# AllenNeuralDynamics/aind-smartspim-destripe

Hardware: AMD Instinct MI355X
Metric: 2048x2048 uint16 slices/s destriped (higher is better)
Workload: dtype f32

## Files before the change

### aind_smartspim_destripe_amd/csrc/dsx.hip

```cpp
#include <hip/hip_runtime.h>
#include <dlfcn.h>
#include <math.h>
#include <rccl/rccl.h>
#include <stdio.h>
#include <stdlib.h>
#include <string.h>

#include <string>
#include <vector>

#include "../../include/dsx.h"
#include "dsx_kernels.h"
#include "dsx_retile.h"
#include "dsx_rot90.h"
#include "dsx_pyramid.h"
#include "dsx_stackrank.h"
#include "dsx_volhist.h"
#include "dsx_project.h"
#include "dsx_wavelet.h"
#include "dsx_plan.h"
#include "dsx_chain.h"
#include "dsx_io.h"
#include "dsx_streaks.h"
#include "dsx_lightsheet.h"
// ... 230 lines not shown
  static bool done[64] = {};
  int dev = 0;
  (void)hipGetDevice(&dev);
  if (done[dev & 63]) return hipSuccess;
  const hipError_t e = hipFuncSetAttribute((const void*)KERN, hipFuncAttributeMaxDynamicSharedMemorySize, (int)bytes);
  if (e == hipSuccess) done[dev & 63] = true;
  return e;
}

template <int CPL, int GF = -1, int NT = -1, int HALO = -1, int PLAN = 0>
hipError_t launch_rowfilter(const DsxTuning& t, const dsx::RowArgs& a, int npairs, int nb, hipStream_t s) {
  if (hipError_t e = raise_lds_limit<dsx::k_rowfilter<CPL, GF, NT, HALO, PLAN>>()) return e;
  const dsx::RowLaunch g = dsx::rowfilter_launch(t, CPL, a.M, npairs);
  hipLaunchKernelGGL((dsx::k_rowfilter<CPL, GF, NT, HALO, PLAN>), dim3(g.grid_x, nb), dim3(64 * g.wpb), g.lds, s, a);
  return hipGetLastError();
}

hipError_t launch_rowfilter_wide(const dsx::RowArgs& a, int npairs, int nb, hipStream_t s) {
  if (hipError_t e = raise_lds_limit<dsx::k_rowfilter_wide>(dsx::kWideMaxLen * sizeof(float2))) return e;
  if (a.M > dsx::kWideMaxLen || a.w >= 65536) return hipErrorInvalidValue;
  hipLaunchKernelGGL(dsx::k_rowfilter_wide, dim3(npairs, nb), dim3(dsx::kWideThreads), (size_t)a.M * sizeof(float2), s, a);
  return hipGetLastError();
}

template <int ID>
hipError_t launch_rowfilter_plan(const DsxTuning& t, const dsx::RowArgs& a, int npairs, int nb, hipStream_t s) {
  constexpr dsx::RowPlan p = dsx::row_plan(ID);
  return launch_rowfilter<p.cpl, p.gf, p.nt, p.halo, ID>(t, a, npairs, nb, s);
}

hipError_t dispatch_rowfilter(const DsxTuning& t, const dsx::RowArgs& a, int npairs, int nb, hipStream_t s) {
  const dsx::RowClass c = dsx::classify_row(a.M, a.w, a.K, a.npass, a.radix);
  if (c.wide) return launch_rowfilter_wide(a, npairs, nb, s);
  switch (c.cpl) {
    case 2: return launch_rowfilter<2>(t, a, npairs, nb, s);
    case 4: return launch_rowfilter<4>(t, a, npairs, nb, s);
    case 6: return launch_rowfilter<6>(t, a, npairs, nb, s);
    case 10: return launch_rowfilter<10>(t, a, npairs, nb, s);
    case 18:
      if (c.plan == 1) return launch_rowfilter_plan<1>(t, a, npairs, nb, s);
      if (c.gf == 4) return launch_rowfilter<18, 4, 1, 0>(t, a, npairs, nb, s);
      if (c.plan == 2) return launch_rowfilter_plan<2>(t, a, npairs, nb, s);
      if (c.gf == 2) return launch_rowfilter<18, 2, 1, 1>(t, a, npairs, nb, s);
      if (c.plan == 5) return launch_rowfilter_plan<5>(t, a, npairs, nb, s);
      if (c.plan == 6) return launch_rowfilter_plan<6>(t, a, npairs, nb, s);
      return launch_rowfilter<18>(t, a, npairs, nb, s);
    default:
      if (c.plan == 3) return launch_rowfilter_plan<3>(t, a, npairs, nb, s);
      if (c.plan == 4) return launch_rowfilter_plan<4>(t, a, npairs, nb, s);
      return launch_rowfilter<36>(t, a, npairs, nb, s);
  }
}

template <int ID>
hipError_t launch_rowfinal_plan(const dsx::RowFinalArgs& a, int nb, hipStream_t s) {
  constexpr dsx::RowPlan p = dsx::row_plan(ID);
  constexpr auto kernel = dsx::k_rowfinal<p.cpl, p.gf, p.nt, p.halo, ID>;
  if (hipError_t e = raise_lds_limit<kernel>()) return e;
  const dsx::RowLaunch g = dsx::rowfinal_launch(a.r.M, a.f.hout);
  hipLaunchKernelGGL(kernel, dim3(g.grid_x, nb), dim3(64 * g.wpb), g.lds, s, a);
  return hipGetLastError();
}

hipError_t launch_rowfinal(int plan, const dsx::RowFinalArgs& a, int nb, hipStream_t s) {
  if (plan == 1) return launch_rowfinal_plan<1>(a, nb, s);
  if (plan == 3) return launch_rowfinal_plan<3>(a, nb, s);
  if (plan == 4) return launch_rowfinal_plan<4>(a, nb, s);
  return hipErrorInvalidValue;
}

hipError_t launch_rowfilter_multi(const dsx::RowMultiArgs& a_in, const int* npairs, int nb, hipStream_t s) {
  if (hipError_t e = raise_lds_limit<dsx::k_rowfilter_multi<6>>()) return e;
  dsx::RowMultiArgs a = a_in;
  int M[dsx::kRowMultiMax];
  for (int i = 0; i < a.nlev; ++i) M[i] = a.lv[i].M;
  const dsx::RowLaunch g = dsx::row_multi_launch(a.nlev, npairs, M, a.blk_end);
  hipLaunchKernelGGL(dsx::k_rowfilter_multi<6>, dim3(g.grid_x, nb), dim3(64 * g.wpb), g.lds, s, a);
  return hipGetLastError();
}

hipError_t launch_rowfilter_pack(const DsxTuning& t, const dsx::RowMultiArgs& m, const int* npairs, int nb, hipStream_t s) {
  if (hipError_t e = raise_lds_limit<dsx::k_rowfilter_pack<6>>()) return e;
  dsx::RowPackArgs a;
  memset(&a, 0, sizeof(a));
  a.nlev = m.nlev;
  int M[dsx::kRowMultiMax];
  for (int i = 0; i < m.nlev; ++i) {
    a.lv[i] = m.lv[i];
    M[i] = m.lv[i].M;
    a.pack[i] = dsx::row_pack_factor(t, m.lv[i].M, m.lv[i].npass, m.lv[i].radix);
  }
  const dsx::RowLaunch g = dsx::row_pack_launch(t, a.nlev, npairs, M, a.pack, a.blk_end);
  hipLaunchKernelGGL(dsx::k_rowfilter_pack<6>, dim3(g.grid_x, nb), dim3(64 * g.wpb), g.lds, s, a);
  return hipGetLastError();
}

struct Chain {
  dsx_ctx* ctx;
  const CohortView& v;
  dsx::ChainShape sh;
  const void* d_in;
  int in_dtype, nb;
  void* d_out;
  int out_dtype;
};

struct Skips {
  int hist, row, from;
};
Skips skips(const DsxTuning& t) {
#ifdef DSX_DIAG
// ... 273 lines not shown
    a.out_plane_stride = (long long)p.Hout * p.Wout;
    a.hout = p.Hout; a.wout = p.Wout;
    a.out_dtype = (c.out_dtype == DSX_U16) ? 0 : 1;
    a.flat = ctx->d_flat;
    a.dark = ctx->d_dark;
    a.dark_ld = ctx->dark_w;
  }
}

int stage_inverse(const Chain& c, const dsx::RowArgs& row1) {
  dsx_ctx* ctx = c.ctx;
  const dsx::Plan& p = ctx->plan;
  const CohortView& v = c.v;
  const dsx::ChainShape& sh = c.sh;
  hipStream_t s = v.stream;
  const int L = p.L, nb = c.nb;
  for (int l = L - 1; l >= (L > 0 ? 0 : -1); --l) {
    if (sh.fuse21 && l == 1) continue;
    if (l >= skips(ctx->tune).from) continue;
    const bool last = (l <= 0);
    LaunchScope ls(ctx, last ? KC_FINAL : KC_INV);
    if (sh.generic) {
      dsx::GenInvArgs g;
      fill_inv(g, c, l);
      g.F = ctx->wl_len;
      memcpy(g.lo, ctx->wl[2], sizeof(float) * ctx->wl_len);
      memcpy(g.hi, ctx->wl[3], sizeof(float) * ctx->wl_len);
      const dim3 gg((g.wout + dsx::kGenOW - 1) / dsx::kGenOW, (g.hout + dsx::kGenOH - 1) / dsx::kGenOH, nb);
      auto kern = level_kernel(last, c.in_dtype, dsx::k_inv_gen<2>, dsx::k_inv_gen<0>, dsx::k_inv_gen<1>);
      hipLaunchKernelGGL(kern, gg, dim3(256), dsx::gen_inv_lds_bytes(g.F), s, g);
      DSX_HIP(hipGetLastError());
      continue;
    }
    dsx::FinalArgs f;
    fill_inv(f, c, l);
    if (!last) f.ws_out = v.ws;
    f.ablate = ctx->ablate;
    const dsx::MarchLaunch m = dsx::inv_launch(sh, ctx->tune, ctx->cus, nb, l, f.hout, f.wout);
    f.nstrips = m.nstrips; f.nseg = m.nseg; f.rows_per_seg = m.rows_per_seg;
    const bool fused = sh.fuse21 && last;
    if (last && sh.split_inv) DSX_HIP(hipStreamWaitEvent(s, v.ev[3], 0));
    if (fused) {
      const dsx::LevelPlan& l2 = p.lv[1];
      f.c2_off = l2.aa_off; f.d2_off = l2.da_off;
      f.hc2 = l2.h; f.wc2 = l2.w; f.ldc2 = l2.lda; f.ldd2 = l2.ld;
      f.has_c2 = (L > 2) ? 1 : 0;
      f.has_c = 1;
      f.pair_io = sh.pair_io ? 1 : 0;
    }
    if (fused && sh.rf_plan != 0) {
      dsx::RowFinalArgs rf;
      rf.r = row1;
      rf.f = f;
      DSX_HIP(launch_rowfinal(sh.rf_plan, rf, nb, s));
      continue;
    }
    auto kern = (fused && m.wpb == 8) ? pixel_kernel(c.in_dtype, dsx::k_inv_march<0, true, 8>, dsx::k_inv_march<1, true, 8>)
                : fused ? pixel_kernel(c.in_dtype, dsx::k_inv_march<0, true>, dsx::k_inv_march<1, true>)
                : level_kernel(last, c.in_dtype, dsx::k_inv_march<2>, dsx::k_inv_march<0>, dsx::k_inv_march<1>);
    hipLaunchKernelGGL(kern, dim3(m.grid_x, nb), dim3(64 * m.wpb), 0, s, f);
    DSX_HIP(hipGetLastError());
  }
  return DSX_OK;
}

int run_cohort(dsx_ctx* ctx, const CohortView& v, const void* d_in, int in_dtype, int nb, void* d_out,
               int out_dtype, int32_t* d_cfg_used) {
  dsx::ChainCall call;
  call.in_u16 = in_dtype == DSX_U16;
  call.out_u16 = out_dtype == DSX_U16;
  call.nb = nb;
  call.aligned16 = (((uintptr_t)d_in | (uintptr_t)d_out) & 15) == 0;
  call.bank = ctx->wl_len > 0;
  call.stop_after = ctx->stop_after;
  call.st_march = ctx->st_march;
  call.has_helper = v.helper != nullptr;
  call.alone = v.alone;
  const Chain c = {ctx, v, dsx::chain_shape(ctx->plan, ctx->tune, call), d_in, in_dtype, nb, d_out, out_dtype};
  if (int rc = stage_zero(c)) return rc;
  if (int rc = stage_forward(c)) return rc;
  if (int rc = stage_thresholds(c, d_cfg_used)) return rc;
  if (ctx->stop_after == 1) return DSX_OK;
  dsx::RowArgs row1;
  if (int rc = stage_rowfilters(c, &row1)) return rc;
  if (ctx->stop_after == 2) return DSX_OK;
  return stage_inverse(c, row1);
}

size_t elem_size(int dtype) { return dtype == DSX_U16 ? 2 : 4; }

int check_run_args(dsx_ctx* ctx, const void* in, const void* out, int n, int in_dtype, int out_dtype) {
  if (n < 0 || (n > 0 && (!in || !out))) return fail(ctx, DSX_EINVAL, "bad plane pointers / count");
  if ((in_dtype != DSX_U16 && in_dtype != DSX_F32) || (out_dtype != DSX_U16 && out_dtype != DSX_F32))
    return fail(ctx, DSX_EINVAL, "unknown element type");
  return DSX_OK;
}

int grow_stage(dsx_ctx* ctx, void** buf, size_t* have, size_t need) {
  if (*have >= need) return DSX_OK;
  if (*buf) (void)hipFree(*buf);
  *buf = nullptr; *have = 0;
  DSX_HIP(hipMalloc(buf, need));
  *have = need;
  return DSX_OK;
}

// ... 434 lines not shown
  if (int rc = check_run_args(ctx, in, out, n, in_dtype, out_dtype)) return rc;
  DSX_HIP(hipSetDevice(ctx->device));
  const size_t in_plane = (size_t)H * W * elem_size(in_dtype);
  const size_t out_plane = (size_t)H * W * elem_size(out_dtype);
  if (host) {
    if (int rc = grow_stage(ctx, &ctx->d_stage_in, &ctx->stage_in_bytes, in_plane * B)) return rc;
    if (int rc = grow_stage(ctx, &ctx->d_stage_out, &ctx->stage_out_bytes, out_plane * B)) return rc;
  }
  if (ctx->rot)
    if (int rc = grow_rot(ctx, in_plane * B, out_plane * B)) return rc;
  auto cohort = [&](const void* d_src, int nb, void* d_dst) -> int {
    if (!ctx->rot) return run_one(ctx, d_src, in_dtype, nb, d_dst, out_dtype);
    rot_planes(use_main(ctx), d_src, ctx->rot_in, in_dtype, nb, ctx->rot_H, ctx->rot_W, +1);
    if (int rc = run_one(ctx, ctx->rot_in, in_dtype, nb, ctx->rot_out, out_dtype)) return rc;
    rot_planes(use_main(ctx), ctx->rot_out, d_dst, out_dtype, nb, H, W, -1);
    DSX_HIP(hipGetLastError());
    return DSX_OK;
  };
  if (host) {
    DSX_HIP(hipStreamSynchronize(use_main(ctx)));
    if (int rc = check_sticky(ctx)) return rc;
  }
  for (int start = 0; start < n; start += B) {
    const int nb = std::min(B, n - start);
    const char* src = (const char*)in + start * in_plane;
    char* dst = (char*)out + start * out_plane;
    if (host) {
      DSX_HIP(hipMemcpyAsync(ctx->d_stage_in, src, in_plane * nb, hipMemcpyHostToDevice, use_main(ctx)));
      if (int rc = cohort(ctx->d_stage_in, nb, ctx->d_stage_out)) return rc;
      DSX_HIP(hipMemcpyAsync(dst, ctx->d_stage_out, out_plane * nb, hipMemcpyDeviceToHost, use_main(ctx)));
      DSX_HIP(hipStreamSynchronize(use_main(ctx)));
      if (ctx->h_sticky && __atomic_exchange_n(ctx->h_sticky, 0u, __ATOMIC_ACQ_REL) != 0u)
        return fail(ctx, DSX_EVALUE, "a plane of " + std::to_string(start) + " .. " + std::to_string(start + nb - 1) +
                                         ": autodetected range of [nan, nan] is not finite (a pixel is NaN, infinite "
                                         "or <= -1)");
    } else if (int rc = cohort(src, nb, dst)) {
      return rc;
    }
  }
  return DSX_OK;
}

int streaks_run(dsx_ctx* ctx, const void* in, int in_dtype, int n, void* out, int out_dtype, bool host) {
  return cohort_run(ctx, ctx->sp.H, ctx->sp.W, ctx->sp.B, streaks_cohort, in, in_dtype, n, out, out_dtype, host);
}

int lightsheet_run(dsx_ctx* ctx, const void* in, int in_dtype, int n, void* out, int out_dtype, bool host) {
  if (in_dtype != DSX_U16) return fail(ctx, DSX_EINVAL, "the light-sheet plan takes uint16 planes only");
  return cohort_run(ctx, ctx->ls_H, ctx->ls_W, ctx->max_batch, lightsheet_cohort, in, in_dtype, n, out, out_dtype, host);
}

}

extern "C" {

int dsx_device_count(void) {
  int n = 0;
  if (hipGetDeviceCount(&n) != hipSuccess) return 0;
  return n;
}

const char* dsx_last_error(const dsx_ctx* ctx) { return ctx ? ctx->err.c_str() : g_init_error.c_str(); }

int dsx_init(int device, dsx_ctx** out_ctx) {
  if (!out_ctx) { g_init_error = "out_ctx is NULL"; return DSX_EINVAL; }
  *out_ctx = nullptr;
  int n = 0;
  hipError_t e = hipGetDeviceCount(&n);
  if (e != hipSuccess || n <= 0) {
    g_init_error = std::string("no HIP device available: ") + hipGetErrorString(e);
    return DSX_EHIP;
  }
  if (device < 0 || device >= n) { g_init_error = "device index out of range"; return DSX_EINVAL; }
  e = hipSetDevice(device);
  if (e != hipSuccess) { g_init_error = std::string("hipSetDevice: ") + hipGetErrorString(e); return DSX_EHIP; }
  dsx_ctx* c = new dsx_ctx();
  c->device = device;
  dsx::read_tuning(c->tune);
  int cus = 0;
  if (hipDeviceGetAttribute(&cus, hipDeviceAttributeMultiprocessorCount, device) == hipSuccess && cus > 0) c->cus = cus;
#ifdef DSX_DIAG
  if (const char* ab = getenv("DSX_ABLATE")) c->ablate = atoi(ab);
#endif
  if (const char* gm = getenv("DSX_GRAPH")) c->graph_mode = atoi(gm) != 0 ? 1 : 0;
  if (const char* ns = getenv("DSX_STREAMS")) c->n_streams = std::max(1, std::min(atoi(ns), (int)dsx_ctx::kMaxStreams));
  int prio[dsx_ctx::kMaxStreams] = {};
  if (const char* pr = getenv("DSX_PRIO")) {
    int i = 0;
    for (const char* q = pr; *q && i < dsx_ctx::kMaxStreams; ++i) {
      prio[i] = atoi(q);
      while (*q && *q != ',') ++q;
      if (*q == ',') ++q;
    }
  }
  e = hipStreamCreateWithPriority(&c->stream_, hipStreamNonBlocking, prio[0]);
  for (int i = 1; i < dsx_ctx::kMaxStreams && e == hipSuccess; ++i) {
    e = hipStreamCreateWithPriority(&c->aux[i], hipStreamNonBlocking, prio[i]);
    if (e == hipSuccess) e = hipEventCreateWithFlags(&c->ev_join[i], hipEventDisableTiming);
  }
  if (e == hipSuccess) e = hipEventCreateWithFlags(&c->ev_fork, hipEventDisableTiming);
  for (int i = 0; i < 2 && e == hipSuccess; ++i) e = hipStreamCreateWithFlags(&c->copy_stream[i], hipStreamNonBlocking);
  for (int i = 0; i < dsx_ctx::kMaxStreams && e == hipSuccess; ++i) {
    e = hipStreamCreateWithFlags(&c->helper[i], hipStreamNonBlocking);
    for (int k = 0; k < 4 && e == hipSuccess; ++k) e = hipEventCreateWithFlags(&c->ev_h[i][k], hipEventDisableTiming);
  }
  if (e == hipSuccess) e = hipEventCreateWithFlags(&c->ev_xs, hipEventDisableTiming);
  for (int i = 0; i < dsx_ctx::kEventSlots && e == hipSuccess; ++i)
    e = hipEventCreateWithFlags(&c->ev_slot[i], hipEventDisableTiming);
  if (e == hipSuccess) e = hipHostMalloc((void**)&c->h_sticky, 64, hipHostMallocMapped);
  if (e == hipSuccess) {
    *c->h_sticky = 0u;
    e = hipHostGetDevicePointer((void**)&c->d_sticky, c->h_sticky, 0);
  }
  if (e == hipSuccess) e = hipEventCreate(&c->t0);
  if (e == hipSuccess) e = hipEventCreate(&c->t1);
  if (e != hipSuccess) {
    g_init_error = std::string("stream/event creation: ") + hipGetErrorString(e);
    delete c;
    return DSX_EHIP;
  }
  *out_ctx = c;
  return DSX_OK;
}

void dsx_destroy(dsx_ctx* ctx) {
  if (!ctx) return;
  (void)hipSetDevice(ctx->device);
  (void)hipStreamSynchronize(use_main(ctx));
  (void)dsx_comm_destroy(ctx);
  for (auto& r : ctx->prof) { (void)hipEventDestroy(r.e0); (void)hipEventDestroy(r.e1); }
  free_plan_buffers(ctx);
  free_streaks(ctx);
  free_lightsheet(ctx);
  if (ctx->t0) (void)hipEventDestroy(ctx->t0);
  if (ctx->t1) (void)hipEventDestroy(ctx->t1);
// ... 1697 lines not shown
```

### aind_smartspim_destripe_amd/csrc/dsx_kernels.h

```cpp
#ifndef DSX_KERNELS_H
#define DSX_KERNELS_H

#include <type_traits>
#include <hip/hip_runtime.h>
#include <stdint.h>

#include "dsx_chain.h"
#include "dsx_fft_core.h"

#ifdef DSX_DIAG
#define DSX_ABL(a, bits) (((a).ablate & (bits)) != 0)
#else
#define DSX_ABL(a, bits) false
#endif

namespace dsx {

constexpr int kMaxLevels = 16;
constexpr int kMaxPasses = 16;
constexpr int kWave = 64;

#define DSX_DEC_LO                                                                              \
  {0.03522629188570953f, -0.08544127388202666f, -0.13501102001025458f, 0.45987750211849154f,   \
   0.8068915093110925f,  0.33267055295008263f}
// ... 1172 lines not shown
struct SlotMask { typedef unsigned long long type; };
template <> struct SlotMask<4> { typedef unsigned type; };
template <> struct SlotMask<8> { typedef unsigned type; };
template <> struct SlotMask<12> { typedef unsigned type; };
template <> struct SlotMask<20> { typedef unsigned type; };

template <int GV, typename F>
__device__ __forceinline__ void for_slots(int gf, int nt, F&& f) {
#pragma unroll
  for (int g = 0; g < GV; ++g) {
    if (g < gf) {
#pragma unroll
      for (int i = 0; i < 4; ++i) f(4 * g + i);
    }
  }
#pragma unroll
  for (int k = 0; k < 4; ++k) {
    if (k < nt) f(4 * GV + k);
  }
}

template <int GV, int E>
__device__ __forceinline__ unsigned count_below_pk16(const unsigned (&x)[E], unsigned t, int gf, int nt) {
  const dsx_s16x2 tv = as_s16x2(t);
  dsx_s16x2 acc = as_s16x2(0u);
  for_slots<GV>(gf, nt, [&](int e) {
    const dsx_s16x2 d = __builtin_elementwise_sub_sat(as_s16x2(x[e]), tv);
    acc -= (d >> 15);
  });
  return as_u32(acc);
}

template <int GV, int E>
__device__ __forceinline__ unsigned bisect_pk16(const unsigned (&x)[E], unsigned rank_a, unsigned rank_b,
                                                int gf, int nt) {
  unsigned ra = 0, rb = 0;
  for (int bit = 15; bit >= 0; --bit) {
    const unsigned ta = ra | (1u << bit), tb = rb | (1u << bit);
    unsigned c = count_below_pk16<GV, E>(x, (ta | (tb << 16)) ^ 0x80008000u, gf, nt);
    c = __reduce_add_sync(~0ull, c);
    if ((c & 0xFFFFu) <= rank_a) ra = ta;
    if ((c >> 16) <= rank_b) rb = tb;
  }
  return ra | (rb << 16);
}

template <int CPL>
constexpr int row_waves_per_simd() {
  return CPL <= 18 ? 4 : 1;
}

__host__ __device__ __forceinline__ constexpr int rf_lds_row_b(int M) { return (M + 1) & ~1; }

template <int CPL, int GF_, int NT_, int HALO_, int PLAN_, bool TO_LDS>
__device__ __forceinline__ void rf_pair_body(const RowArgs& a, float2* s_tw, float2* buf, int tid, int nthreads, int lane,
                                             int pair, int plane) {
  const int M = (PLAN_ > 0) ? StaticFft<PLAN_>::M : a.M;
  constexpr bool SWZ = StaticFft<PLAN_>::kSwz;
  auto P = [](int i) { return SWZ ? dsx_idx_swz::at(i) : i; };
  const int N = a.w, K = (HALO_ == 0) ? 0 : a.K;
  const bool halo = (HALO_ >= 0) ? (HALO_ != 0) : (K > 0);
  const int npairs = (a.h + 1) >> 1;
  const bool live = pair < npairs;
  const int r0 = live ? 2 * pair : 0;
  const bool has_b = (r0 + 1) < a.h;
  const int cfg = a.cfg[plane];
  float* rowa = a.ws + plane * a.ws_plane_stride + a.da_off + (long long)r0 * a.ld;
  float* rowb = rowa + a.ld;

  constexpr int GV = RowSlots<CPL>::GV;
  constexpr int E = RowSlots<CPL>::E;
  typedef typename SlotMask<E>::type mask_t;
  const int gf = (GF_ >= 0) ? GF_ : (N >> 8);
  const int tail0 = gf << 8;
  const int nt = (NT_ >= 0) ? NT_ : ((N - tail0 + 63) >> 6);
  const int tn = tail0 + lane;

  const bool inactive = a.lvl >= a.lvl_active[cfg];
  auto zero_rows = [&]() {
    if (live) {
      for (int n = 4 * lane; n < N; n += 4 * kWave) {
        *(float4*)(rowa + n) = make_float4(0.f, 0.f, 0.f, 0.f);
        if (has_b) *(float4*)(rowb + n) = make_float4(0.f, 0.f, 0.f, 0.f);
      }
    }
  };
  if (!TO_LDS && inactive) {
    zero_rows();
    return;
  }
  const bool active = live && !inactive;
  const float thr = a.thr[(long long)plane * a.L + a.lvl];

  float4 ra4[GV > 0 ? GV : 1], rb4[GV > 0 ? GV : 1];
  float rta[4], rtb[4];
#pragma unroll
  for (int g = 0; g < GV; ++g) {
    ra4[g] = make_float4(0.f, 0.f, 0.f, 0.f);
    rb4[g] = make_float4(0.f, 0.f, 0.f, 0.f);
    if (active && g < gf) {
      ra4[g] = *(const float4*)(rowa + 256 * g + 4 * lane);
      if (has_b) rb4[g] = *(const float4*)(rowb + 256 * g + 4 * lane);
    }
  }
#pragma unroll
  for (int k = 0; k < 4; ++k) {
    rta[k] = 0.f;
    rtb[k] = 0.f;
    if (active && k < nt && tn + 64 * k < N) {
      rta[k] = rowa[tn + 64 * k];
      if (has_b) rtb[k] = rowb[tn + 64 * k];
    }
  }
  for (int i = tid; i < M; i += nthreads) s_tw[P(i)] = a.tw[i];
  __syncthreads();
  float* const lds_a = (float*)buf;
  float* const lds_b = (float*)buf + rf_lds_row_b(M);
  if (!active) {
    if (TO_LDS) {
      for (int n = 2 * lane; n < N; n += 2 * kWave) {
        *(float2*)(lds_a + n) = make_float2(0.f, 0.f);
        *(float2*)(lds_b + n) = make_float2(0.f, 0.f);
      }
    }
    return;
  }

  float va[E], vb[E];
  mask_t maska = 0, maskb = 0;
  auto take = [&](int e, float xa, float xb, bool valid) {
    const bool ma = valid && fabsf(xa) > thr, mb = valid && fabsf(xb) > thr;
    if (ma) maska |= ((mask_t)1 << e);
    if (mb) maskb |= ((mask_t)1 << e);
    va[e] = valid ? (ma ? 0.f : xa) : __builtin_huge_valf();
    vb[e] = valid ? (mb ? 0.f : xb) : __builtin_huge_valf();
  };
#pragma unroll
  for (int g = 0; g < GV; ++g) {
    if (g < gf) {
      take(4 * g + 0, ra4[g].x, rb4[g].x, true);
      take(4 * g + 1, ra4[g].y, rb4[g].y, true);
      take(4 * g + 2, ra4[g].z, rb4[g].z, true);
      take(4 * g + 3, ra4[g].w, rb4[g].w, true);
    }
  }
#pragma unroll
  for (int k = 0; k < 4; ++k) {
    if (k < nt) take(4 * GV + k, rta[k], rtb[k], tn + 64 * k < N);
  }
  if (!has_b) {
    for_slots<GV>(gf, nt, [&](int e) { if (vb[e] != __builtin_huge_valf()) vb[e] = 0.f; });
  }

  float meda = 0.f, medb = 0.f;
  const bool any_mask = __ballot((maska | maskb) != (mask_t)0) != 0ull;
  if (any_mask && !DSX_ABL(a, 1)) {
    const unsigned k1 = (unsigned)(N - 1) >> 1;
    const bool even = (N & 1) == 0;
    auto count2 = [&](float ta, float tb, bool le) -> unsigned {
      unsigned ca = 0, cb = 0;
      for_slots<GV>(gf, nt, [&](int e) {
        ca += (unsigned)__popcll(__ballot(le ? (va[e] <= ta) : (va[e] < ta)));
        cb += (unsigned)__popcll(__ballot(le ? (vb[e] <= tb) : (vb[e] < tb)));
      });
      return ca | (cb << 16);
    };
    float lo[2], hi[2];
    unsigned clo[2], chi[2];
    bool done[2];
    float flo[2], fhi[2];
    int last[2] = {0, 0};
    const float target = (float)k1 + 0.5f;
    const float thr_up = as_f32(as_u32(thr) + 1u);
    {
      const unsigned c0 = count2(0.f, 0.f, false), c0e = count2(0.f, 0.f, true);
#pragma unroll
// ... 43 lines not shown
      }
    }
    float m_lo[2] = {__builtin_huge_valf(), __builtin_huge_valf()}, m_hi[2] = {__builtin_huge_valf(), __builtin_huge_valf()};
    for_slots<GV>(gf, nt, [&](int e) {
      m_lo[0] = min_no_nan(m_lo[0], va[e] >= lo[0] ? va[e] : __builtin_huge_valf());
      m_lo[1] = min_no_nan(m_lo[1], vb[e] >= lo[1] ? vb[e] : __builtin_huge_valf());
      if (even) {
        m_hi[0] = min_no_nan(m_hi[0], va[e] >= hi[0] ? va[e] : __builtin_huge_valf());
        m_hi[1] = min_no_nan(m_hi[1], vb[e] >= hi[1] ? vb[e] : __builtin_huge_valf());
      }
    });
    float sk[2], sk1[2];
#pragma unroll
    for (int r = 0; r < 2; ++r) {
      sk[r] = wave_min_no_nan(m_lo[r]);
      sk1[r] = sk[r];
      if (even) {
        const float nxt = wave_min_no_nan(m_hi[r]);
        sk1[r] = (k1 + 1u < chi[r]) ? sk[r] : nxt;
      }
    }
    meda = even ? 0.5f * (sk[0] + sk1[0]) : sk[0];
    medb = even ? 0.5f * (sk[1] + sk1[1]) : sk[1];
  }
  asm volatile("" : "+v"(meda), "+v"(medb));

  for_slots<GV>(gf, nt, [&](int e) {
    const int n = (e < 4 * GV) ? 256 * (e >> 2) + 4 * lane + (e & 3) : tn + 64 * (e - 4 * GV);
    if (e < 4 * GV || n < N) {
      const float xa = bit_select(slot_mask(maska, e), meda, va[e]);
      const float xb = bit_select(slot_mask(maskb, e), medb, vb[e]);
      const float2 z = make_float2(xa, xb);
      buf[P(K + n)] = z;
      if (halo) {
        if (n <= K) buf[P(K + N + n)] = z;
        if (n >= N - K) buf[P(n - (N - K))] = z;
      }
    }
  });
  if (halo) {
    for (int m = N + 2 * K + 1 + lane; m < M; m += kWave) buf[P(m)] = make_float2(0.f, 0.f);
  }
  wave_sync();

  if (!DSX_ABL(a, 2)) {
    if constexpr (PLAN_ > 0) StaticFft<PLAN_>::template run_forward<CPL>(buf, s_tw, lane, a.kcut[cfg]);
    else fft_run<CPL>(buf, s_tw, a, lane);
  }

  if (!DSX_ABL(a, 4)) {
    const float2* g1 = a.g[cfg];
    const float2* g2 = g1 + M;
    const int kcut = a.kcut[cfg];
    for (int k = lane; k <= kcut; k += kWave) {
      const int kr = (k == 0) ? 0 : M - k;
      const float2 u = buf[P(k)], ur = buf[P(kr)];
      const float ga = g1[k].x;
      const float2 gb = g2[k];
      const float2 v = make_float2(ga * u.x + gb.x * ur.x - gb.y * ur.y, ga * u.y + gb.x * ur.y + gb.y * ur.x);
      const float2 vr = make_float2(ga * ur.x + gb.x * u.x + gb.y * u.y, ga * ur.y + gb.x * u.y - gb.y * u.x);
      buf[P(k)] = make_float2(v.y, v.x);
      if (kr != k) buf[P(kr)] = make_float2(vr.y, vr.x);
    }
    for (int k = kcut + 1 + lane; k < M - kcut; k += kWave) buf[P(k)] = make_float2(0.f, 0.f);
    wave_sync();
  }

  if (!DSX_ABL(a, 2)) {
    if constexpr (PLAN_ > 0) StaticFft<PLAN_>::template run_inverse<CPL>(buf, s_tw, lane, a.kcut[cfg]);
    else fft_run<CPL>(buf, s_tw, a, lane);
  }

  maska = opaque_mask(maska);
  maskb = opaque_mask(maskb);
  if (TO_LDS) {
    float oa[E], ob[E];
    const int no_b = has_b ? 0 : -1;
    for_slots<GV>(gf, nt, [&](int e) {
      const int n = (e < 4 * GV) ? 256 * (e >> 2) + 4 * lane + (e & 3) : tn + 64 * (e - 4 * GV);
      oa[e] = 0.f;
      ob[e] = 0.f;
      if (e < 4 * GV || n < N) {
        const float2 y = buf[P(K + n)];
        oa[e] = bit_select(slot_mask(maska, e), 0.f, -y.y * a.inv_M);
        ob[e] = bit_select(slot_mask(maskb, e) | no_b, 0.f, -y.x * a.inv_M);
      }
    });
    wave_sync();
#pragma unroll
    for (int g = 0; g < GV; ++g) {
      if (g < gf) {
        const int nb0 = 256 * g + 4 * lane;
        *(float2*)(lds_a + nb0) = make_float2(oa[4 * g], oa[4 * g + 1]);
        *(float2*)(lds_a + nb0 + 2) = make_float2(oa[4 * g + 2], oa[4 * g + 3]);
        *(float2*)(lds_b + nb0) = make_float2(ob[4 * g], ob[4 * g + 1]);
        *(float2*)(lds_b + nb0 + 2) = make_float2(ob[4 * g + 2], ob[4 * g + 3]);
      }
    }
#pragma unroll
    for (int k = 0; k < 4; ++k) {
      const int n = tn + 64 * k;
      if (k < nt && n < N) {
        lds_a[n] = oa[4 * GV + k];
        lds_b[n] = ob[4 * GV + k];
      }
    }
    return;
  }
#pragma unroll
  for (int g = 0; g < GV; ++g) {
    if (g < gf) {
      const int nb0 = 256 * g + 4 * lane;
      float da_[4], db_[4];
#pragma unroll
      for (int i = 0; i < 4; ++i) {
        const int e = 4 * g + i;
        const float2 y = buf[P(K + nb0 + i)];
        da_[i] = bit_select(slot_mask(maska, e), 0.f, -y.y * a.inv_M);
        db_[i] = bit_select(slot_mask(maskb, e), 0.f, -y.x * a.inv_M);
      }
      const dsx_f4 oa = {da_[0], da_[1], da_[2], da_[3]}, ob = {db_[0], db_[1], db_[2], db_[3]};
      __builtin_nontemporal_store(oa, (dsx_f4*)(rowa + nb0));
      if (has_b) __builtin_nontemporal_store(ob, (dsx_f4*)(rowb + nb0));
    }
  }
#pragma unroll
  for (int k = 0; k < 4; ++k) {
    const int n = tn + 64 * k;
    if (k < nt && n < N) {
      const int e = 4 * GV + k;
      const float2 y = buf[P(K + n)];
      rowa[n] = bit_select(slot_mask(maska, e), 0.f, -y.y * a.inv_M);
      if (has_b) rowb[n] = bit_select(slot_mask(maskb, e), 0.f, -y.x * a.inv_M);
    }
  }
}

template <int CPL, int GF_ = -1, int NT_ = -1, int HALO_ = -1, int PLAN_ = 0>
__global__ __launch_bounds__(64 * kRowMaxWaves, row_waves_per_simd<CPL>()) void k_rowfilter(RowArgs a) {
  extern __shared__ __attribute__((aligned(16))) float2 dsx_smem[];
  const int tid = threadIdx.x, lane = tid & 63, wave = tid >> 6;
  const int M = (PLAN_ > 0) ? StaticFft<PLAN_>::M : a.M;
  rf_pair_body<CPL, GF_, NT_, HALO_, PLAN_, false>(a, dsx_smem, dsx_smem + (long long)M * (1 + wave), tid, blockDim.x, lane,
                                                   blockIdx.x * (blockDim.x >> 6) + wave, blockIdx.y);
}

struct RowMultiArgs {
  int nlev;
  int blk_end[kRowMultiMax];
  RowArgs lv[kRowMultiMax];
};

template <int CPL>
__global__ __launch_bounds__(64 * kRowMaxWaves, row_waves_per_simd<CPL>()) void k_rowfilter_multi(RowMultiArgs args) {
  extern __shared__ __attribute__((aligned(16))) float2 dsx_smem[];
  const int tid = threadIdx.x, lane = tid & 63, wave = tid >> 6;
  int ent = 0;
  while (ent + 1 < args.nlev && (int)blockIdx.x >= args.blk_end[ent]) ++ent;
  const RowArgs& a = args.lv[ent];
// ... 960 lines not shown
      ni[2] = issue_i(2 * (p + 3) + 2);
      ni[3] = issue_i(2 * (p + 3) + 3);
    }
    if (p + 2 < p_end) step(p + 2, nc[2], ni[4], ni[5], A[2], A[0], A[1], D[2], D[0], D[1]);
    if (more) {
      nc[2] = issue_c(p + 7);
      ni[4] = issue_i(2 * (p + 3) + 4);
      ni[5] = issue_i(2 * (p + 3) + 5);
    }
  }
}

constexpr int kInvMinWaves = 1;
template <int IN_KIND, bool FUSE = false, int WPB = 4>
__global__ __launch_bounds__(64 * WPB, (FUSE && IN_KIND == 0) ? kInvMinWaves : 1) void k_inv_march(FinalArgs a) {
  __shared__ __attribute__((aligned(16))) float s_c1[FUSE ? WPB : 1][FUSE ? kRingRows : 1][FUSE ? kC1Pitch : 4];
  const int lane = threadIdx.x & 63;
  const int wave = __builtin_amdgcn_readfirstlane(threadIdx.x >> 6);
  const int item = blockIdx.x * WPB + wave;
  if (item >= a.nstrips * a.nseg) return;
  const int strip = item % a.nstrips, seg = item / a.nstrips;
  const int plane = blockIdx.y;
  if (seg * a.rows_per_seg >= ((a.hout + 1) >> 1)) return;
  const int x0 = kMarchCols * strip + 4 * lane;
  if (FUSE) {
    float (*ring)[kC1Pitch] = (float (*)[kC1Pitch])s_c1[wave];
    const bool pair = IN_KIND == 0 && a.pair_io != 0;
    if (IN_KIND == 0 && pair) {
      if (a.flat != nullptr) inv_march_body<IN_KIND, true, true, true, IN_KIND == 0>(a, lane, strip, seg, plane, ring);
      else inv_march_body<IN_KIND, true, false, true, IN_KIND == 0>(a, lane, strip, seg, plane, ring);
      return;
    }
    if (a.flat != nullptr) inv_march_body<IN_KIND, true, true, true>(a, lane, strip, seg, plane, ring);
    else inv_march_body<IN_KIND, true, false, true>(a, lane, strip, seg, plane, ring);
    return;
  }
  if (x0 >= a.wout) return;
  const bool lane_fast = (a.has_pyr != 0) && ((a.ldc & 1) == 0) && ((a.ldd & 1) == 0) &&
                         (IN_KIND == 2 || (((a.W & 3) == 0) && (x0 + 3 < a.W)));
  const bool fast = __all(lane_fast) != 0;
  if (IN_KIND != 2 && a.flat != nullptr) {
    if (fast) inv_march_body<IN_KIND, true, IN_KIND != 2>(a, lane, strip, seg, plane);
    else inv_march_body<IN_KIND, false, IN_KIND != 2>(a, lane, strip, seg, plane);
  } else {
    if (fast) inv_march_body<IN_KIND, true, false>(a, lane, strip, seg, plane);
    else inv_march_body<IN_KIND, false, false>(a, lane, strip, seg, plane);
  }
}


struct RowFinalArgs {
  RowArgs r;
  FinalArgs f;
};

struct RowFinalPre {
  uint4 ni[2];

};

template <bool SHADE, bool STEADY_, bool PREFETCH_ONLY = false>
__device__ __forceinline__ void rowfinal_synth(const FinalArgs& a, const float2* smem, int M, int lane, int strip, int plane,
                                               int p_begin, int p_end, int row0, RowFinalPre& pre) {
  constexpr float RL0[6] = DSX_REC_LO;
  constexpr float RH0[6] = DSX_REC_HI;
  constexpr float KS = 1.44269504088896340736f;
  constexpr float RL[6] = {RL0[0] * KS, RL0[1] * KS, RL0[2] * KS, RL0[3] * KS, RL0[4] * KS, RL0[5] * KS};
  constexpr float RH[6] = {RH0[0] * KS, RH0[1] * KS, RH0[2] * KS, RH0[3] * KS, RH0[4] * KS, RH0[5] * KS};
  constexpr bool STEADY = STEADY_ && !SHADE;
  const int x0 = kMarchCols * strip + 4 * lane;
  const int xl = min(x0, a.W - 4);
  const int ql = xl >> 1;
  const bool odd_lane = (lane & 1) != 0;
  const int oddm = odd_lane_mask(lane);
  const int xb = min(kMarchCols * strip + 8 * (lane >> 1), a.W - 8);
  const __amdgpu_buffer_rsrc_t rs_img = dsx_rsrc((const char*)a.img + plane * a.img_plane_stride * 2);
  const long long out_bytes = (long long)a.hout * a.wout * 2;
  const __amdgpu_buffer_rsrc_t rs_out =
      STEADY ? dsx_rsrc_bounded((const char*)a.out + plane * a.out_plane_stride * 2, (unsigned)min(out_bytes, (long long)kBufDiscard))
             : dsx_rsrc((const char*)a.out + plane * a.out_plane_stride * 2);
  const unsigned vo_pair0 = (unsigned)xb * 2u, vo_pair = vo_pair0 + (odd_lane ? (unsigned)a.W * 2u : 0u);
  const unsigned vo_pair_out = (unsigned)xb * 2u + (odd_lane ? (unsigned)a.wout * 2u : 0u);
  const unsigned vo_store = x0 < a.wout ? vo_pair_out : kBufDiscard;
  const int store_rows = a.hout - (odd_lane ? 1 : 0);
  const int xs = min(x0, max(a.wout - 4, 0));
  const __amdgpu_buffer_rsrc_t rs_dark = dsx_rsrc(SHADE ? a.dark : a.ws), rs_flat = dsx_rsrc(SHADE ? a.flat : a.ws);
  const unsigned vo_shade = (unsigned)xs * 4u;
  const bool shade_vec = SHADE && (a.wout & 3) == 0 && (a.dark_ld & 3) == 0 && a.wout >= 4 &&
                         (((uintptr_t)a.dark | (uintptr_t)a.flat) & 15) == 0;

  const int Q = ql >> 1;
  const float* c2base = a.ws + plane * a.ws_plane_stride + a.c2_off;
  const float* d2base = a.ws + plane * a.ws_plane_stride + a.d2_off;
  const __amdgpu_buffer_rsrc_t rs_c2 = STEADY ? dsx_rsrc_bounded(c2base, a.has_c2 ? kBufDiscard : 0u) : dsx_rsrc(c2base);
  const __amdgpu_buffer_rsrc_t rs_d2 = dsx_rsrc(d2base);
  const unsigned vo_2 = (unsigned)Q * 4u;
  auto l2_load = [&](int P2) {
    FinalRawC r;
    r.c01 = r.c23 = make_float2(0.f, 0.f);
    const int pr = min(P2, a.hc2 - 1);
    if (STEADY || a.has_c2) {
      const dsx_u32x4 u = __builtin_amdgcn_raw_buffer_load_b128(rs_c2, vo_2, (unsigned)(pr * a.ldc2) * 4u, 0);
      r.c01 = make_float2(__uint_as_float(u.x), __uint_as_float(u.y));
      r.c23 = make_float2(__uint_as_float(u.z), __uint_as_float(u.w));
    }
    const dsx_u32x4 u = __builtin_amdgcn_raw_buffer_load_b128(rs_d2, vo_2, (unsigned)(pr * a.ldd2) * 4u, 0);
    r.d01 = make_float2(__uint_as_float(u.x), __uint_as_float(u.y));
    r.d23 = make_float2(__uint_as_float(u.z), __uint_as_float(u.w));
    return r;
  };
  const int gy_last = STEADY ? min(2 * p_end - 2, a.H - 1) : a.H - 1;
  auto issue_i = [&](int gy) {
    const int ge = min(gy, gy_last);
    const unsigned vo = (ge + 1 < a.H) ? vo_pair : vo_pair0;
    const dsx_u32x4 u = __builtin_amdgcn_raw_buffer_load_b128(rs_img, vo, (unsigned)(ge * a.W) * 2u, kBufNT);
    return make_uint4(u.x, u.y, u.z, u.w);
// ... 1 lines not shown
  int next_P = p_begin >> 1, c1_ready = p_begin;
  if (PREFETCH_ONLY) {
#pragma unroll
    for (int r = 0; r < 2; ++r) pre.ni[r] = issue_i(2 * (p_begin + r));
    return;
  }
  dsx_f2 A2[3][2], D2[3][2];
  dsx_f2 c1e[2], c1o[2];
  {
    const FinalRawC w0 = l2_load(next_P), w1 = l2_load(next_P + 1);
    final_xsynth(w0.c01, w0.c23, A2[0]);
    final_xsynth(w0.d01, w0.d23, D2[0]);
    final_xsynth(w1.c01, w1.c23, A2[1]);
    final_xsynth(w1.d01, w1.d23, D2[1]);
  }
  FinalRawC n2 = l2_load(next_P + 2);
  auto l2_step = [&]() {
    final_xsynth(n2.c01, n2.c23, A2[2]);
    final_xsynth(n2.d01, n2.d23, D2[2]);
    n2 = l2_load(next_P + 3);
#pragma unroll
    for (int h = 0; h < 2; ++h) {
      c1e[h] = pk_dot6(A2[0][h], RL0[4], A2[1][h], RL0[2], A2[2][h], RL0[0], D2[0][h], RH0[4], D2[1][h], RH0[2],
                       D2[2][h], RH0[0]);
      c1o[h] = pk_dot6(A2[0][h], RL0[5], A2[1][h], RL0[3], A2[2][h], RL0[1], D2[0][h], RH0[5], D2[1][h], RH0[3],
                       D2[2][h], RH0[1]);
      A2[0][h] = A2[1][h]; A2[1][h] = A2[2][h];
      D2[0][h] = D2[1][h]; D2[1][h] = D2[2][h];
    }
    ++next_P;
    c1_ready += 2;
  };
  auto c1_row = [&](auto par, int p, dsx_f2 (&out)[2]) {
    constexpr int PAR = decltype(par)::value;
    if constexpr (PAR < 0) {
      if (c1_ready <= p) l2_step();
    } else if constexpr (PAR == 0) {
      l2_step();
    }
    const bool odd = PAR < 0 ? (p & 1) != 0 : PAR != 0;
    const dsx_f2 lo = odd ? c1o[0] : c1e[0], hi = odd ? c1o[1] : c1e[1];
    final_xsynth(make_float2(lo.x, lo.y), make_float2(hi.x, hi.y), out);
  };
  using RowEven = std::integral_constant<int, STEADY ? 0 : -1>;
  using RowOdd = std::integral_constant<int, STEADY ? 1 : -1>;
  using AtRunTime = std::integral_constant<int, -1>;
  auto d1_row = [&](int r, dsx_f2 (&out)[2]) {
    const int rr = r - row0;
    const float* row = (const float*)(smem + (long long)M * (1 + (rr >> 1))) + ((rr & 1) ? rf_lds_row_b(M) : 0) + ql;
    const float2 lo = *(const float2*)row, hi = *(const float2*)(row + 2);
    final_xsynth(lo, hi, out);
  };

  dsx_f2 A[3][2], D[3][2];
  uint4 ni[3] = {pre.ni[0], pre.ni[1], issue_i(2 * (p_begin + 2))};
  c1_row(RowEven(), p_begin, A[0]);
  d1_row(p_begin, D[0]);
  c1_row(RowOdd(), p_begin + 1, A[1]);
  d1_row(p_begin + 1, D[1]);

  auto px_row = [&](auto vec, int gy, uint2 u, const dsx_f2 (&c0p)[2], unsigned (&pk)[2]) {
    const float c0[4] = {c0p[0].x, c0p[0].y, c0p[1].x, c0p[1].y};
    const float px[4] = {(float)(u.x & 0xFFFFu), (float)(u.x >> 16), (float)(u.y & 0xFFFFu), (float)(u.y >> 16)};
    float r[4];
    if (SHADE) {
      float dk[4], fl[4];
      const int gys = min(gy, a.hout - 1);
      if (decltype(vec)::value < 0 ? shade_vec : decltype(vec)::value != 0) {
        const dsx_u32x4 d4 = __builtin_amdgcn_raw_buffer_load_b128(rs_dark, vo_shade, (unsigned)(gys * a.dark_ld) * 4u, 0);
        const dsx_u32x4 f4 = __builtin_amdgcn_raw_buffer_load_b128(rs_flat, vo_shade, (unsigned)(gys * a.wout) * 4u, 0);
        dk[0] = __uint_as_float(d4.x); dk[1] = __uint_as_float(d4.y); dk[2] = __uint_as_float(d4.z); dk[3] = __uint_as_float(d4.w);
        fl[0] = __uint_as_float(f4.x); fl[1] = __uint_as_float(f4.y); fl[2] = __uint_as_float(f4.z); fl[3] = __uint_as_float(f4.w);
      } else {
#pragma unroll
        for (int e = 0; e < 4; ++e) {
          const int gx = min(x0 + e, a.wout - 1);
          dk[e] = a.dark[(long long)gys * a.dark_ld + gx];
          fl[e] = a.flat[(long long)gys * a.wout + gx];
        }
      }
#pragma unroll
      for (int e = 0; e < 4; ++e) r[e] = final_px<SHADE>(a, c0[e], px[e], dk[e], fl[e]);
    } else {
#pragma unroll
      for (int h = 0; h < 2; ++h) {
        const dsx_f2 one = {1.0f, 1.0f};
        const dsx_f2 x1 = dsx_f2{px[2 * h], px[2 * h + 1]} + one;
        const dsx_f2 ex = {__builtin_amdgcn_exp2f(c0[2 * h]), __builtin_amdgcn_exp2f(c0[2 * h + 1])};
        const dsx_f2 v = pk_fma(x1, ex, one);
        r[2 * h] = v.x;
        r[2 * h + 1] = v.y;
      }
    }
    pk[0] = pack_u16_sat(r[0], r[1]);
    pk[1] = pack_u16_sat(r[2], r[3]);
  };
  auto step = [&](auto par, auto vec, int p, const uint4& ri, dsx_f2 (&A0)[2], dsx_f2 (&A1)[2], dsx_f2 (&A2w)[2],
                  dsx_f2 (&D0)[2], dsx_f2 (&D1)[2], dsx_f2 (&D2w)[2]) {
    c1_row(par, p + 2, A2w);
    d1_row(p + 2, D2w);
    dsx_f2 even[2], odd[2];
#pragma unroll
    for (int h = 0; h < 2; ++h) {
      even[h] = pk_dot6(A0[h], RL[4], A1[h], RL[2], A2w[h], RL[0], D0[h], RH[4], D1[h], RH[2], D2w[h], RH[0]);
      odd[h] = pk_dot6(A0[h], RL[5], A1[h], RL[3], A2w[h], RL[1], D0[h], RH[5], D1[h], RH[3], D2w[h], RH[1]);
    }
    const unsigned sx = bit_select(oddm, ri.x, ri.z), sy = bit_select(oddm, ri.y, ri.w);
    const unsigned gx = swap_adjacent(sx), gyv = swap_adjacent(sy);
    const uint2 r0 = make_uint2(bit_select(oddm, gx, ri.x), bit_select(oddm, gyv, ri.y));
    const uint2 r1 = make_uint2(bit_select(oddm, ri.z, gx), bit_select(oddm, ri.w, gyv));
    unsigned pe[2], po[2];
    px_row(vec, 2 * p, r0, even, pe);
    px_row(vec, 2 * p + 1, r1, odd, po);
    const unsigned tx = swap_adjacent(bit_select(oddm, pe[0], po[0])), ty = swap_adjacent(bit_select(oddm, pe[1], po[1]));
    dsx_u32x4 o4;
    o4.x = bit_select(oddm, tx, pe[0]);
    o4.y = bit_select(oddm, ty, pe[1]);
    o4.z = bit_select(oddm, po[0], tx);
    o4.w = bit_select(oddm, po[1], ty);
    if constexpr (decltype(par)::value >= 0) {
      const unsigned vo = 2 * p < store_rows ? vo_store : kBufDiscard;
      __builtin_amdgcn_raw_buffer_store_b128(o4, rs_out, vo, (unsigned)(2 * p * a.wout) * 2u, kBufNT);
      __builtin_amdgcn_sched_barrier(0);
      asm volatile("s_nop 2");
      __builtin_amdgcn_sched_barrier(0);
    } else {
      const int gyl = 2 * p + (odd_lane ? 1 : 0);
      if (gyl < a.hout && x0 < a.wout)
        __builtin_amdgcn_raw_buffer_store_b128(o4, rs_out, vo_pair_out, (unsigned)(2 * p * a.wout) * 2u, kBufNT);
    }
  };
  if constexpr (STEADY) {
    const std::integral_constant<int, 1> vec;
    for (int p = p_begin;; p += 6) {
      step(RowEven(), vec, p, ni[0], A[0], A[1], A[2], D[0], D[1], D[2]);
      ni[0] = issue_i(2 * (p + 3));
      step(RowOdd(), vec, p + 1, ni[1], A[1], A[2], A[0], D[1], D[2], D[0]);
      ni[1] = issue_i(2 * (p + 4));
      if (p + 2 >= p_end) break;
      step(RowEven(), vec, p + 2, ni[2], A[2], A[0], A[1], D[2], D[0], D[1]);
      ni[2] = issue_i(2 * (p + 5));
      step(RowOdd(), vec, p + 3, ni[0], A[0], A[1], A[2], D[0], D[1], D[2]);
      ni[0] = issue_i(2 * (p + 6));
      if (p + 4 >= p_end) break;
      step(RowEven(), vec, p + 4, ni[1], A[1], A[2], A[0], D[1], D[2], D[0]);
      ni[1] = issue_i(2 * (p + 7));
      step(RowOdd(), vec, p + 5, ni[2], A[2], A[0], A[1], D[2], D[0], D[1]);
      ni[2] = issue_i(2 * (p + 8));
      if (p + 6 >= p_end) break;
    }
  } else {
    const AtRunTime rt;
    for (int p = p_begin; p < p_end; p += 3) {
      const bool more = p + 3 < p_end;
      step(rt, rt, p, ni[0], A[0], A[1], A[2], D[0], D[1], D[2]);
      if (more) ni[0] = issue_i(2 * (p + 3));
      if (p + 1 < p_end) step(rt, rt, p + 1, ni[1], A[1], A[2], A[0], D[1], D[2], D[0]);
      if (more) ni[1] = issue_i(2 * (p + 4));
      if (p + 2 < p_end) step(rt, rt, p + 2, ni[2], A[2], A[0], A[1], D[2], D[0], D[1]);
      if (more) ni[2] = issue_i(2 * (p + 5));
    }
  }
}

template <int CPL, int GF_, int NT_, int HALO_, int PLAN_>
__global__ __launch_bounds__(64 * kRfWaves, CPL <= 18 ? 4 : 2) void k_rowfinal(RowFinalArgs a) {
  extern __shared__ __attribute__((aligned(16))) float2 dsx_smem[];
  const int tid = threadIdx.x, lane = tid & 63;
  const int wave = __builtin_amdgcn_readfirstlane(tid >> 6);
  constexpr int M = StaticFft<PLAN_>::M;
  const int plane = blockIdx.y;
  const int bx = blockIdx.x;
  const int pair0 = (kRfWaves - 1) * bx;
  rf_pair_body<CPL, GF_, NT_, HALO_, PLAN_, true>(a.r, dsx_smem, dsx_smem + (long long)M * (1 + wave), tid, 64 * kRfWaves, lane,
                                                  pair0 + wave, plane);
  const int np = (a.f.hout + 1) >> 1;
  const int p_begin = 2 * pair0, p_end = min(np, p_begin + kRfRows);
  const bool synth = wave < a.f.nstrips && p_begin < p_end;
  RowFinalPre pre;
  asm volatile("" ::: "memory");
  __builtin_amdgcn_sched_barrier(0);
  constexpr bool STEADY = CPL <= 18;
  if (synth) rowfinal_synth<false, STEADY, true>(a.f, dsx_smem, M, lane, wave, plane, p_begin, p_end, 2 * pair0, pre);
  __syncthreads();
  if (!synth) return;
  if (a.f.flat != nullptr) rowfinal_synth<true, STEADY>(a.f, dsx_smem, M, lane, wave, plane, p_begin, p_end, 2 * pair0, pre);
  else rowfinal_synth<false, STEADY>(a.f, dsx_smem, M, lane, wave, plane, p_begin, p_end, 2 * pair0, pre);
}

}
#endif
```

Measured before the change: 72670.

## Replace block barrier in rowfinal with per-wave LDS ready flags and stage gains in LDS

Removes the __syncthreads between the per-wave row-filter phase and the synthesis phase of the fused rowfinal kernel. In its place, each wave publishes an LDS ready flag, and consumer waves spin on only the neighbour pairs they need, so filtering and synthesis can overlap across waves. It also copies the band gains into a shared LDS handover struct when kcut is small, replacing global loads, and lowers the dynamic LDS limit to leave room for that struct. The risks are spin-wait cost, correctness of the hand-rolled LDS flag ordering, and less LDS headroom. DSX_DIAG-only timing counters are added as well.

After: 73050 (median of 6 runs). No clear change (+0.5%).

```diff
diff --git a/aind_smartspim_destripe_amd/csrc/dsx.hip b/aind_smartspim_destripe_amd/csrc/dsx.hip
--- a/aind_smartspim_destripe_amd/csrc/dsx.hip
+++ b/aind_smartspim_destripe_amd/csrc/dsx.hip
@@ -306,11 +306,15 @@
   }
 }
 
+#ifdef DSX_DIAG
+unsigned long long* g_rowfinal_diag = nullptr;
+#endif
+
 template <int ID>
 hipError_t launch_rowfinal_plan(const dsx::RowFinalArgs& a, int nb, hipStream_t s) {
   constexpr dsx::RowPlan p = dsx::row_plan(ID);
   constexpr auto kernel = dsx::k_rowfinal<p.cpl, p.gf, p.nt, p.halo, ID>;
-  if (hipError_t e = raise_lds_limit<kernel>()) return e;
+  if (hipError_t e = raise_lds_limit<kernel>(dsx::kLdsLimit - sizeof(dsx::RfHandover))) return e;
   const dsx::RowLaunch g = dsx::rowfinal_launch(a.r.M, a.f.hout);
   hipLaunchKernelGGL(kernel, dim3(g.grid_x, nb), dim3(64 * g.wpb), g.lds, s, a);
   return hipGetLastError();
@@ -690,6 +694,9 @@
       dsx::RowFinalArgs rf;
       rf.r = row1;
       rf.f = f;
+#ifdef DSX_DIAG
+      rf.diag = g_rowfinal_diag;
+#endif
       DSX_HIP(launch_rowfinal(sh.rf_plan, rf, nb, s));
       continue;
     }
@@ -1230,6 +1237,15 @@
 
 }
 
+#ifdef DSX_DIAG
+extern "C" int dsx_diag_rowfinal(unsigned long long* out8) {
+  if (g_rowfinal_diag == nullptr) return DSX_EINVAL;
+  if (hipDeviceSynchronize() != hipSuccess) return DSX_EHIP;
+  if (hipMemcpy(out8, g_rowfinal_diag, 64, hipMemcpyDeviceToHost) != hipSuccess) return DSX_EHIP;
+  return hipMemset(g_rowfinal_diag, 0, 64) == hipSuccess ? DSX_OK : DSX_EHIP;
+}
+#endif
+
 extern "C" {
 
 int dsx_device_count(void) {
@@ -1259,6 +1275,7 @@
   if (hipDeviceGetAttribute(&cus, hipDeviceAttributeMultiprocessorCount, device) == hipSuccess && cus > 0) c->cus = cus;
 #ifdef DSX_DIAG
   if (const char* ab = getenv("DSX_ABLATE")) c->ablate = atoi(ab);
+  if (g_rowfinal_diag == nullptr && hipMalloc(&g_rowfinal_diag, 64) == hipSuccess) (void)hipMemset(g_rowfinal_diag, 0, 64);
 #endif
   if (const char* gm = getenv("DSX_GRAPH")) c->graph_mode = atoi(gm) != 0 ? 1 : 0;
   if (const char* ns = getenv("DSX_STREAMS")) c->n_streams = std::max(1, std::min(atoi(ns), (int)dsx_ctx::kMaxStreams));
diff --git a/aind_smartspim_destripe_amd/csrc/dsx_kernels.h b/aind_smartspim_destripe_amd/csrc/dsx_kernels.h
--- a/aind_smartspim_destripe_amd/csrc/dsx_kernels.h
+++ b/aind_smartspim_destripe_amd/csrc/dsx_kernels.h
@@ -1248,9 +1248,31 @@
 
 __host__ __device__ __forceinline__ constexpr int rf_lds_row_b(int M) { return (M + 1) & ~1; }
 
+constexpr int kRfGains = 208;
+struct RfHandover {
+  unsigned ready[kRfWaves];
+  float g1[kRfGains];
+  float2 g2[kRfGains];
+};
+typedef __attribute__((address_space(3))) unsigned dsx_lds_u32;
+__device__ __forceinline__ void rf_publish(RfHandover* ho, int slot) {
+  asm volatile("s_waitcnt lgkmcnt(0)" ::: "memory");
+  *(volatile dsx_lds_u32*)&ho->ready[slot] = 1u;
+}
+__device__ __forceinline__ void rf_await(const RfHandover* ho, int slot) {
+  const unsigned flag = (unsigned)(uintptr_t)(const dsx_lds_u32*)&ho->ready[slot];
+#pragma unroll 1
+  for (int spins = 0; spins < (1 << 24); ++spins) {
+    unsigned v = flag;
+    asm volatile("ds_read_b32 %0, %0\n\ts_waitcnt lgkmcnt(0)" : "+v"(v)::"memory");
+    if (__builtin_expect(__builtin_amdgcn_readfirstlane(v) != 0u, 1)) break;
+    __builtin_amdgcn_s_sleep(2);
+  }
+}
+
 template <int CPL, int GF_, int NT_, int HALO_, int PLAN_, bool TO_LDS>
 __device__ __forceinline__ void rf_pair_body(const RowArgs& a, float2* s_tw, float2* buf, int tid, int nthreads, int lane,
-                                             int pair, int plane) {
+                                             int pair, int plane, RfHandover* ho = nullptr, int slot = 0) {
   const int M = (PLAN_ > 0) ? StaticFft<PLAN_>::M : a.M;
   constexpr bool SWZ = StaticFft<PLAN_>::kSwz;
   auto P = [](int i) { return SWZ ? dsx_idx_swz::at(i) : i; };
@@ -1309,6 +1331,18 @@
     }
   }
   for (int i = tid; i < M; i += nthreads) s_tw[P(i)] = a.tw[i];
+  const bool lds_gains = TO_LDS && a.kcut[cfg] < kRfGains;
+  if constexpr (TO_LDS) {
+    if (lds_gains) {
+      const float2* g1 = a.g[cfg];
+      const float2* g2 = g1 + M;
+      for (int k = tid; k <= a.kcut[cfg]; k += nthreads) {
+        ho->g1[k] = g1[k].x;
+        ho->g2[k] = g2[k];
+      }
+    }
+    if (tid < kRfWaves) ho->ready[tid] = 0u;
+  }
   __syncthreads();
   float* const lds_a = (float*)buf;
   float* const lds_b = (float*)buf + rf_lds_row_b(M);
@@ -1318,6 +1352,7 @@
         *(float2*)(lds_a + n) = make_float2(0.f, 0.f);
         *(float2*)(lds_b + n) = make_float2(0.f, 0.f);
       }
+      rf_publish(ho, slot);
     }
     return;
   }
@@ -1467,16 +1502,20 @@
     const float2* g1 = a.g[cfg];
     const float2* g2 = g1 + M;
     const int kcut = a.kcut[cfg];
-    for (int k = lane; k <= kcut; k += kWave) {
-      const int kr = (k == 0) ? 0 : M - k;
-      const float2 u = buf[P(k)], ur = buf[P(kr)];
-      const float ga = g1[k].x;
-      const float2 gb = g2[k];
-      const float2 v = make_float2(ga * u.x + gb.x * ur.x - gb.y * ur.y, ga * u.y + gb.x * ur.y + gb.y * ur.x);
-      const float2 vr = make_float2(ga * ur.x + gb.x * u.x + gb.y * u.y, ga * ur.y + gb.x * u.y - gb.y * u.x);
-      buf[P(k)] = make_float2(v.y, v.x);
-      if (kr != k) buf[P(kr)] = make_float2(vr.y, vr.x);
-    }
+    auto band = [&](auto gain1, auto gain2) {
+      for (int k = lane; k <= kcut; k += kWave) {
+        const int kr = (k == 0) ? 0 : M - k;
+        const float2 u = buf[P(k)], ur = buf[P(kr)];
+        const float ga = gain1(k);
+        const float2 gb = gain2(k);
+        const float2 v = make_float2(ga * u.x + gb.x * ur.x - gb.y * ur.y, ga * u.y + gb.x * ur.y + gb.y * ur.x);
+        const float2 vr = make_float2(ga * ur.x + gb.x * u.x + gb.y * u.y, ga * ur.y + gb.x * u.y - gb.y * u.x);
+        buf[P(k)] = make_float2(v.y, v.x);
+        if (kr != k) buf[P(kr)] = make_float2(vr.y, vr.x);
+      }
+    };
+    if (lds_gains) band([&](int k) { return ho->g1[k]; }, [&](int k) { return ho->g2[k]; });
+    else band([&](int k) { return g1[k].x; }, [&](int k) { return g2[k]; });
     for (int k = kcut + 1 + lane; k < M - kcut; k += kWave) buf[P(k)] = make_float2(0.f, 0.f);
     wave_sync();
   }
@@ -1520,6 +1559,7 @@
         lds_b[n] = ob[4 * GV + k];
       }
     }
+    rf_publish(ho, slot);
     return;
   }
 #pragma unroll
@@ -2586,16 +2626,30 @@
 struct RowFinalArgs {
   RowArgs r;
   FinalArgs f;
+#ifdef DSX_DIAG
+  unsigned long long* diag;
+#endif
 };
 
 struct RowFinalPre {
   uint4 ni[2];
-
+#ifdef DSX_DIAG
+  unsigned long long waited = 0;
+#endif
 };
+#ifdef DSX_DIAG
+__device__ __forceinline__ unsigned long long rf_stamp() {
+  unsigned long long t;
+  __builtin_amdgcn_sched_barrier(0);
+  asm volatile("s_memtime %0\n\ts_waitcnt lgkmcnt(0)" : "=s"(t)::"memory");
+  __builtin_amdgcn_sched_barrier(0);
+  return t;
+}
+#endif
 
 template <bool SHADE, bool STEADY_, bool PREFETCH_ONLY = false>
 __device__ __forceinline__ void rowfinal_synth(const FinalArgs& a, const float2* smem, int M, int lane, int strip, int plane,
-                                               int p_begin, int p_end, int row0, RowFinalPre& pre) {
+                                               int p_begin, int p_end, int row0, RowFinalPre& pre, const RfHandover* ho) {
   constexpr float RL0[6] = DSX_REC_LO;
   constexpr float RH0[6] = DSX_REC_HI;
   constexpr float KS = 1.44269504088896340736f;
@@ -2703,8 +2757,20 @@
     final_xsynth(lo, hi, out);
   };
 
+  auto await_pair = [&](int s) {
+#ifdef DSX_DIAG
+    const unsigned long long t0 = rf_stamp();
+#endif
+    rf_await(ho, s);
+#ifdef DSX_DIAG
+    pre.waited += rf_stamp() - t0;
+#endif
+  };
+
   dsx_f2 A[3][2], D[3][2];
   uint4 ni[3] = {pre.ni[0], pre.ni[1], issue_i(2 * (p_begin + 2))};
+  await_pair(0);
+  await_pair(1);
   c1_row(RowEven(), p_begin, A[0]);
   d1_row(p_begin, D[0]);
   c1_row(RowOdd(), p_begin + 1, A[1]);
@@ -2748,6 +2814,11 @@
   };
   auto step = [&](auto par, auto vec, int p, const uint4& ri, dsx_f2 (&A0)[2], dsx_f2 (&A1)[2], dsx_f2 (&A2w)[2],
                   dsx_f2 (&D0)[2], dsx_f2 (&D1)[2], dsx_f2 (&D2w)[2]) {
+    if constexpr (decltype(par)::value == 0) {
+      await_pair((p + 2 - row0) >> 1);
+    } else if constexpr (decltype(par)::value < 0) {
+      if (((p - row0) & 1) == 0) await_pair((p + 2 - row0) >> 1);
+    }
     c1_row(par, p + 2, A2w);
     d1_row(p + 2, D2w);
     dsx_f2 even[2], odd[2];
@@ -2823,8 +2894,12 @@
   const int plane = blockIdx.y;
   const int bx = blockIdx.x;
   const int pair0 = (kRfWaves - 1) * bx;
+  __shared__ RfHandover s_ho;
+#ifdef DSX_DIAG
+  const unsigned long long t_start = rf_stamp();
+#endif
   rf_pair_body<CPL, GF_, NT_, HALO_, PLAN_, true>(a.r, dsx_smem, dsx_smem + (long long)M * (1 + wave), tid, 64 * kRfWaves, lane,
-                                                  pair0 + wave, plane);
+                                                  pair0 + wave, plane, &s_ho, wave);
   const int np = (a.f.hout + 1) >> 1;
   const int p_begin = 2 * pair0, p_end = min(np, p_begin + kRfRows);
   const bool synth = wave < a.f.nstrips && p_begin < p_end;
@@ -2832,12 +2907,25 @@
   asm volatile("" ::: "memory");
   __builtin_amdgcn_sched_barrier(0);
   constexpr bool STEADY = CPL <= 18;
-  if (synth) rowfinal_synth<false, STEADY, true>(a.f, dsx_smem, M, lane, wave, plane, p_begin, p_end, 2 * pair0, pre);
-  __syncthreads();
-  if (!synth) return;
-  if (a.f.flat != nullptr) rowfinal_synth<true, STEADY>(a.f, dsx_smem, M, lane, wave, plane, p_begin, p_end, 2 * pair0, pre);
-  else rowfinal_synth<false, STEADY>(a.f, dsx_smem, M, lane, wave, plane, p_begin, p_end, 2 * pair0, pre);
-}
-
-}
+  if (synth) rowfinal_synth<false, STEADY, true>(a.f, dsx_smem, M, lane, wave, plane, p_begin, p_end, 2 * pair0, pre, &s_ho);
+#ifdef DSX_DIAG
+  const unsigned long long t_filtered = rf_stamp();
 #endif
+  if (synth) {
+    if (a.f.flat != nullptr) rowfinal_synth<true, STEADY>(a.f, dsx_smem, M, lane, wave, plane, p_begin, p_end, 2 * pair0, pre, &s_ho);
+    else rowfinal_synth<false, STEADY>(a.f, dsx_smem, M, lane, wave, plane, p_begin, p_end, 2 * pair0, pre, &s_ho);
+  }
+#ifdef DSX_DIAG
+  if (a.diag != nullptr && lane == 0) {
+    unsigned long long* d = a.diag + 4 * a.r.cfg[plane];
+    const unsigned long long t_end = rf_stamp();
+    atomicAdd(d + 0, pre.waited);
+    atomicAdd(d + 1, t_filtered - t_start);
+    atomicAdd(d + 2, t_end - t_start);
+    atomicAdd(d + 3, 1ull);
+  }
+#endif
+}
+
+}
+#endif
```
